# KLab/YAIK

Measured on AMD Instinct MI355X. Metric: Mpix/s tile encode (alpha reject + 7 gradient passes + 8x8 range quant), 8K RGBA, higher is better.
Workload: dtype u8/int32 (+f32 mode-selection sums)

## Files before the change

### yaik_amd/csrc/yk_encode2.hip

```cpp
#include "yk_common.h"
#include "yk_curves.h"
#include "yk_device.h"
#include <mutex>

__constant__ float c_curve2[6][16] = YK_CURVE_TABLE;

#define LS YK_LSTRIDE
#ifdef YK_TEST_HOOKS
#define YK2_ABLATE(bit) ((P.ablate & (bit)) != 0)
#else
#define YK2_ABLATE(bit) false
#endif

__device__ __forceinline__ int y2_byte(uint32_t w, int ch) { return (w >> (8 * ch)) & 255; }
__device__ __forceinline__ uint32_t y2_absdiff(uint32_t a, uint32_t b) { uint32_t r; asm("v_sad_u32 %0, %1, %2, 0" : "=v"(r) : "v"(a), "v"(b)); return r; }
__device__ __forceinline__ int y2_round6(int v) { return (v & ~3) | (v >> 6); }
__device__ __forceinline__ int y2_round6p(int v) { v = min(v + 1, 255); return (v & ~3) | (v >> 6); }

typedef short y2s2 __attribute__((ext_vector_type(2)));
typedef unsigned short y2u2 __attribute__((ext_vector_type(2)));
__device__ __forceinline__ y2u2 y2_u2(uint32_t w) { return __builtin_bit_cast(y2u2, w); }
__device__ __forceinline__ y2s2 y2_s2(y2u2 v) { return __builtin_bit_cast(y2s2, v); }
__device__ __forceinline__ y2u2 y2_splat(int v) { const unsigned short t = (unsigned short)v; return (y2u2){ t, t }; }
__device__ __forceinline__ y2s2 y2_splats(int v) { const short t = (short)v; return (y2s2){ t, t }; }
__device__ __forceinline__ y2s2 y2_rg(uint32_t p) { return y2_s2(y2_u2(__builtin_amdgcn_perm(0u, p, 0x010C000Cu) ^ 0x80008000u)); }
__device__ __forceinline__ y2s2 y2_bb(uint32_t pEven, uint32_t pOdd) { return y2_s2(y2_u2(__builtin_amdgcn_perm(pOdd, pEven, 0x060C020Cu) ^ 0x80008000u)); }
#define YK2_LATN 85
#ifdef YK2_STATS
__device__ unsigned long long g_y2_stats[128];
#define YK2_STAT(i, n) do { if (lane == 0) atomicAdd(&g_y2_stats[(i)], (unsigned long long)(n)); } while (0)
extern "C" int yk_debug_path_stats(unsigned long long* out, int clear) {
    hipError_t e = hipMemcpyFromSymbol(out, HIP_SYMBOL(g_y2_stats), sizeof(g_y2_stats));
    if (e == hipSuccess && clear) { static unsigned long long z[128]; e = hipMemcpyToSymbol(HIP_SYMBOL(g_y2_stats), z, sizeof(z)); }
    return (int)e;
}
#else
#define YK2_STAT(i, n) do { } while (0)
#endif

__device__ __forceinline__ constexpr int y2_cell_x(int m) { return (m & 1) | ((m >> 1) & 2); }
__device__ __forceinline__ constexpr int y2_cell_y(int m) { return ((m >> 1) & 1) | ((m >> 2) & 2); }
template <int NX, int NY> __device__ __forceinline__ constexpr unsigned long long y2_origin() {
    unsigned long long m = 0;
    for (int i = 0; i < 16; i++) if ((y2_cell_x(i) % NX) == 0 && (y2_cell_y(i) % NY) == 0) m |= 1ULL << i;
    return m * 0x0001000100010001ULL;
}
template <int NX, int NY> __device__ __forceinline__ unsigned long long y2_fold(unsigned long long m) {
    if (NX >= 2) m |= m >> 1;
    if (NY >= 2) m |= m >> 2;
    if (NX == 4) m |= m >> 4;
    if (NY == 4) m |= m >> 8;
    return m;
}
template <int NX, int NY> __device__ __forceinline__ unsigned long long y2_spread(unsigned long long m) {
    if (NX >= 2) m |= m << 1;
    if (NY >= 2) m |= m << 2;
    if (NX == 4) m |= m << 4;
    if (NY == 4) m |= m << 8;
    return m;
}

template <int SX, int SY, bool SMOOTH = false>
__device__ __forceinline__ void y2_grad_pass(const uint32_t* s_lat, const int lat, const int cx, const int cy,
                                             const y2s2 (&rg)[16], const y2s2 (&bb)[8], unsigned long long& cov, const unsigned long long deadLanes, const bool stripInside,
                                             const int gxCell, const int gyCell, const int w, const int h, const int rf,
                                             uint32_t* s_bm, const int bxCell, const int byCell, const uint32_t* s_pix, uint8_t* s_list, uint32_t* s_tf, const int lane) {
    constexpr int TX = 1 << SX, TY = 1 << SY, NX = TX / 4, NY = TY / 4;
    constexpr unsigned long long ORG = y2_origin<NX, NY>();
    const int dcx = cx & (NX - 1), dcy = cy & (NY - 1);
    unsigned long long viable = ORG & ~cov & ~y2_fold<NX, NY>(deadLanes);
    if (!stripInside) {
        const int tgx = gxCell - dcx * 4, tgy = gyCell - dcy * 4;
        viable &= __ballot((tgx + TX <= w) && (tgy + TY <= h));
    }
    if (viable == 0ULL) return;
    constexpr int kPassId = (SX == 4 && SY == 4) ? 0 : (SX == 4 && SY == 3) ? 1 : (SX == 3 && SY == 4) ? 2 : (SX == 3 && SY == 3) ? 3 : (SX == 3 && SY == 2) ? 4 : (SX == 2 && SY == 3) ? 5 : 6;
    YK2_STAT(kPassId * 10 + 0, 1); YK2_STAT(kPassId * 10 + 8, __popcll(y2_spread<NX, NY>(viable)));
    const int loO = -256 * rf, hiO = 256 * rf + 255;
    const y2s2 loO2 = y2_splats(loO), hiO2 = y2_splats(hiO), loR2 = y2_splats(loO - 127), hiR2 = y2_splats(hiO - 127);


#ifndef YK2_NO_COMPACT
    const unsigned long long cells = y2_spread<NX, NY>(viable);
    const int nCells = __popcll(cells);
    if (nCells <= 16) {
        YK2_STAT(kPassId * 10 + 1, 1); YK2_STAT(kPassId * 10 + 7, nCells);
        const int rank = (int)__builtin_amdgcn_mbcnt_hi((uint32_t)(cells >> 32), __builtin_amdgcn_mbcnt_lo((uint32_t)cells, 0u));
        const bool mine = __builtin_amdgcn_inverse_ballot_w64(cells);
        if (mine) s_list[rank] = (uint8_t)lane;
        s_tf[lane] = 0u; s_tf[64 + lane] = 0u;
        __builtin_amdgcn_fence(__ATOMIC_RELEASE, "wavefront"); __builtin_amdgcn_wave_barrier(); __builtin_amdgcn_fence(__ATOMIC_ACQUIRE, "wavefront");
        const int j = lane & 15, r = lane >> 4;
        const bool act = j < nCells;
        const int c = (int)s_list[act ? j : 0];
        const int q2 = c >> 4, cy2 = y2_cell_y(c & 15), cx2 = y2_cell_x(c & 15);
        const int dcx2 = cx2 & (NX - 1), dcy2 = cy2 & (NY - 1);
        constexpr int kInTile = (NX > 1 ? 1 : 0) | (NY > 1 ? 2 : 0) | (NX > 2 ? 4 : 0) | (NY > 2 ? 8 : 0);
        const int orig = c & ~kInTile;
        const int lo2 = cy2 * 17 + q2 * 4 + cx2 - dcy2 * 17 - dcx2;
        const y2u2 wyr = y2_splat(16 - ((dcy2 * 4 + r) << (4 - SY)));
        const y2u2 lxc = y2_splat(16 - ((dcx2 * 4) << (4 - SX)));
        const uint4 pr = *reinterpret_cast<const uint4*>(&s_pix[(cy2 * 4 + r) * LS + q2 * 16 + cx2 * 4]);
        const y2s2 rgc[4] = { y2_rg(pr.x), y2_rg(pr.y), y2_rg(pr.z), y2_rg(pr.w) }, bbc[2] = { y2_bb(pr.x, pr.y), y2_bb(pr.z, pr.w) };
        y2s2 mnc[5], mxc[5];
        auto rowC = [&](const unsigned mask) {
            y2u2 Sc[5], stc[5];
#pragma unroll
            for (int t = 0; t < 5; t++) {
                if (!((mask >> t) & 1u)) continue;
                const uint32_t* lt = s_lat + t * YK2_LATN + lo2;
                const y2u2 TL = y2_u2(lt[0]), TR = y2_u2(lt[NX]), BL = y2_u2(lt[NY * 17]), BR = y2_u2(lt[NY * 17 + NX]);
                const y2u2 e16 = (BL - BR) << 4, g = TR - BR, f = TL - BL - g;
                const y2u2 c2 = (g << 4) + f * lxc;
                Sc[t] = ((BR << 8) + e16 * lxc + c2 * wyr) ^ y2_splat(0x8000);
                stc[t] = (e16 + f * wyr) << (4 - SX);
            }
#pragma unroll
            for (int i = 0; i < 4; i++) {
                const y2s2 c01 = rgc[i], cb = bbc[i >> 1];
                const y2s2 cc[4] = { __builtin_shufflevector(c01, c01, 0, 0), __builtin_shufflevector(c01, c01, 1, 1),
                                     (i & 1) ? __builtin_shufflevector(cb, cb, 1, 1) : __builtin_shufflevector(cb, cb, 0, 0), c01 };
#pragma unroll
                for (int t = 0; t < 4; t++) {
                    if (!((mask >> t) & 1u)) continue;
                    const y2s2 D = __builtin_elementwise_sub_sat(y2_s2(Sc[t]), cc[t]);
                    if (i == 0) { mnc[t] = D; mxc[t] = D; }
                    else { mnc[t] = __builtin_elementwise_min(mnc[t], D); mxc[t] = __builtin_elementwise_max(mxc[t], D); }
                    if (i < 3) Sc[t] = Sc[t] - stc[t];
                }
            }
            if (mask & 0x10u) {
                const y2s2 Da = __builtin_elementwise_sub_sat(y2_s2(Sc[4] - stc[4] * (y2u2){ 0, 1 }), bbc[0]);
                const y2s2 Db = __builtin_elementwise_sub_sat(y2_s2(Sc[4] - stc[4] * (y2u2){ 2, 3 }), bbc[1]);
                mnc[4] = __builtin_elementwise_min(Da, Db); mxc[4] = __builtin_elementwise_max(Da, Db);
            }
        };
        constexpr uint32_t kAllFail = 0xE000E000u;
        auto failBits = [&](const y2s2 mnA, const y2s2 mxA, const y2s2 mnP, const y2s2 mxP) -> uint32_t {
            const y2s2 zero = y2_splats(0);
            const y2s2 oA = __builtin_elementwise_sub_sat(zero, __builtin_elementwise_max(__builtin_elementwise_sub_sat(loO2, mnA), __builtin_elementwise_sub_sat(mxA, hiO2)));
            const y2s2 rA = __builtin_elementwise_sub_sat(zero, __builtin_elementwise_max(__builtin_elementwise_sub_sat(loR2, mnA), __builtin_elementwise_sub_sat(mxA, hiR2)));
            const y2s2 oP = __builtin_elementwise_sub_sat(zero, __builtin_elementwise_max(__builtin_elementwise_sub_sat(loO2, mnP), __builtin_elementwise_sub_sat(mxP, hiO2)));
            const y2s2 rP = __builtin_elementwise_sub_sat(zero, __builtin_elementwise_max(__builtin_elementwise_sub_sat(loR2, mnP), __builtin_elementwise_sub_sat(mxP, hiR2)));
            const uint32_t a = __builtin_bit_cast(uint32_t, oA), b = __builtin_bit_cast(uint32_t, rA), cO = __builtin_bit_cast(uint32_t, oP), cR = __builtin_bit_cast(uint32_t, rP);
            uint32_t m = (a & 0x80008000u) | ((b >> 1) & 0x40004000u);
            m |= (((cO << 16) | cO) >> 2) & 0x20000000u;
            m |= (((cR >> 16) | cR) >> 2) & 0x00002000u;
            return m;
        };
        rowC(0x09u);
        if (act) atomicOr(&s_tf[orig], failBits(mnc[0], mxc[0], mnc[3], mxc[3]));
        __builtin_amdgcn_fence(__ATOMIC_RELEASE, "wavefront"); __builtin_amdgcn_wave_barrier(); __builtin_amdgcn_fence(__ATOMIC_ACQUIRE, "wavefront");
        const unsigned long long alive = viable & __ballot(s_tf[lane] != kAllFail);
        if (alive == 0ULL) { YK2_STAT(100 + kPassId, 1); return; }
        rowC(0x16u);
        {
            const y2s2 mnA = __builtin_elementwise_min(__builtin_elementwise_min(mnc[0], mnc[1]), mnc[2]), mxA = __builtin_elementwise_max(__builtin_elementwise_max(mxc[0], mxc[1]), mxc[2]);
            const y2s2 mnP = __builtin_elementwise_min(mnc[3], mnc[4]), mxP = __builtin_elementwise_max(mxc[3], mxc[4]);
            if (act) atomicOr(&s_tf[64 + orig], failBits(mnA, mxA, mnP, mxP));
        }
        __builtin_amdgcn_fence(__ATOMIC_RELEASE, "wavefront"); __builtin_amdgcn_wave_barrier(); __builtin_amdgcn_fence(__ATOMIC_ACQUIRE, "wavefront");
        const unsigned long long acceptC = alive & __ballot(s_tf[64 + lane] != kAllFail);
        if (acceptC != 0ULL) {
            YK2_STAT(110 + kPassId, 1);
            cov |= y2_spread<NX, NY>(acceptC);
            if (__builtin_amdgcn_inverse_ballot_w64(acceptC)) {
                const int tbx = bxCell >> SX, tby = byCell >> SY;
                int bit;
                if (SX == 4 && SY == 4) bit = 0 + tby * 4 + tbx;
                else if (SX == 4 && SY == 3) bit = 32 + tby * 4 + tbx;
                else if (SX == 3 && SY == 4) bit = 64 + tby * 8 + tbx;
                else if (SX == 3 && SY == 3) bit = 96 + tby * 8 + tbx;
                else if (SX == 3 && SY == 2) bit = 160 + (tby >> 3) * 64 + (tby & 7) * 8 + tbx;
                else if (SX == 2 && SY == 3) bit = 288 + (tbx >> 3) * 64 + tby * 8 + (tbx & 7);
                else bit = 416 + ((tby >> 3) * 2 + (tbx >> 3)) * 64 + (tby & 7) * 8 + (tbx & 7);
                atomicOr(&s_bm[bit >> 5], 1u << (bit & 31));
            }
        }
        return;
    }
#endif

    const int lo = lat - dcy * 17 - dcx;
    const y2u2 wy2 = y2_splat(16 - ((dcy * 4) << (4 - SY)));
    const y2u2 lx2 = y2_splat(16 - ((dcx * 4) << (4 - SX)));
    y2u2 S[4], st[4], dS0[4], dS3[4], dst[4], Sa, Sb, rsA, rsB;
    auto setup = [&](const int t) {
        const uint32_t* lt = s_lat + t * YK2_LATN + lo;
        const y2u2 TL = y2_u2(lt[0]), TR = y2_u2(lt[NX]), BL = y2_u2(lt[NY * 17]), BR = y2_u2(lt[NY * 17 + NX]);
        const y2u2 e16 = (BL - BR) << 4, g = TR - BR, f = TL - BL - g;
        const y2u2 c2 = (g << 4) + f * lx2;
        const y2u2 s0 = ((BR << 8) + e16 * lx2 + c2 * wy2) ^ y2_splat(0x8000);
        const y2u2 d0 = c2 << (4 - SY);
        const y2u2 sx = (e16 + f * wy2) << (4 - SX);
        const y2u2 dx = f << (8 - SX - SY);
        if (t < 4) {
            S[t] = s0; dS0[t] = d0; st[t] = sx; dst[t] = dx;
            dS3[t] = d0 - dx * (unsigned short)3;
        } else {
            const y2u2 k01 = { 0, 1 }, k23 = { 2, 3 };
            Sa = s0 - sx * k01; Sb = s0 - sx * k23;
            rsA = d0 - dx * k01; rsB = d0 - dx * k23;
        }
    };
    y2s2 mn[5], mx[5];
    auto pixelRow = [&](const int r, const unsigned mask, const bool first) {
        if (mask & 0x0Fu) {
#pragma unroll
            for (int ii = 0; ii < 4; ii++) {
                const int i = (r & 1) ? 3 - ii : ii;
                const y2s2 c01 = rg[r * 4 + i], cb = bb[r * 2 + (i >> 1)];
                const y2s2 cc[4] = { __builtin_shufflevector(c01, c01, 0, 0), __builtin_shufflevector(c01, c01, 1, 1),
                                     (i & 1) ? __builtin_shufflevector(cb, cb, 1, 1) : __builtin_shufflevector(cb, cb, 0, 0), c01 };
#pragma unroll
                for (int t = 0; t < 4; t++) {
                    if (!((mask >> t) & 1u)) continue;
                    const y2s2 D = __builtin_elementwise_sub_sat(y2_s2(S[t]), cc[t]);
                    if (first && ii == 0) { mn[t] = D; mx[t] = D; }
                    else { mn[t] = __builtin_elementwise_min(mn[t], D); mx[t] = __builtin_elementwise_max(mx[t], D); }
                    if (ii < 3) S[t] = (r & 1) ? S[t] + st[t] : S[t] - st[t];
                }
            }
        }
        if (mask & 0x10u) {
            const y2s2 Da = __builtin_elementwise_sub_sat(y2_s2(Sa), bb[r * 2]), Db = __builtin_elementwise_sub_sat(y2_s2(Sb), bb[r * 2 + 1]);
            const y2s2 lo4 = __builtin_elementwise_min(Da, Db), hi4 = __builtin_elementwise_max(Da, Db);
            if (first) { mn[4] = lo4; mx[4] = hi4; }
            else { mn[4] = __builtin_elementwise_min(mn[4], lo4); mx[4] = __builtin_elementwise_max(mx[4], hi4); }
        }
    };
    auto nextRow = [&](const int r, const unsigned mask) {
#pragma unroll
        for (int t = 0; t < 4; t++) if ((mask >> t) & 1u) { S[t] -= (r & 1) ? dS0[t] : dS3[t]; st[t] -= dst[t]; }
        if (mask & 0x10u) { Sa -= rsA; Sb -= rsB; }
    };
    auto failA4 = [&](const y2s2 mnA, const y2s2 mxA) -> unsigned long long {
        const y2s2 oA = __builtin_elementwise_max(__builtin_elementwise_sub_sat(loO2, mnA), __builtin_elementwise_sub_sat(mxA, hiO2));
        const y2s2 rA = __builtin_elementwise_max(__builtin_elementwise_sub_sat(loR2, mnA), __builtin_elementwise_sub_sat(mxA, hiR2));
        unsigned long long f = y2_fold<NX, NY>(__ballot(oA.x > 0));
        f &= y2_fold<NX, NY>(__ballot(oA.y > 0));
        f &= y2_fold<NX, NY>(__ballot(rA.x > 0));
        f &= y2_fold<NX, NY>(__ballot(rA.y > 0));
        return f;
    };
    auto failP2 = [&](const y2s2 mnP, const y2s2 mxP) -> unsigned long long {
        const y2s2 oP = __builtin_elementwise_max(__builtin_elementwise_sub_sat(loO2, mnP), __builtin_elementwise_sub_sat(mxP, hiO2));
        const y2s2 rP = __builtin_elementwise_max(__builtin_elementwise_sub_sat(loR2, mnP), __builtin_elementwise_sub_sat(mxP, hiR2));
        return y2_fold<NX, NY>(__ballot((oP.x > 0) | (oP.y > 0))) & y2_fold<NX, NY>(__ballot((rP.x > 0) | (rP.y > 0)));
    };
    auto mnAll = [&]() { return __builtin_elementwise_min(__builtin_elementwise_min(mn[0], mn[1]), mn[2]); };
    auto mxAll = [&]() { return __builtin_elementwise_max(__builtin_elementwise_max(mx[0], mx[1]), mx[2]); };

    constexpr bool kScreen = (NX * NY >= 4);
    constexpr unsigned kA = 0x07u, kP = 0x18u;
    unsigned long long accept;
    if (SMOOTH) {
        setup(0); setup(1); setup(2);
        pixelRow(0, kA, true);
        nextRow(0, kA); pixelRow(1, kA, false);
        nextRow(1, kA); pixelRow(2, kA, false);
        nextRow(2, kA); pixelRow(3, kA, false);
// ... 3 lines not shown
        {
            y2u2 S_[4], st_[4], a_[4], b_[4], c_[4]; y2s2 mn_[5], mx_[5];
            for (int t = 0; t < 4; t++) { S_[t] = S[t]; st_[t] = st[t]; a_[t] = dS0[t]; b_[t] = dS3[t]; c_[t] = dst[t]; }
            for (int t = 0; t < 5; t++) { mn_[t] = mn[t]; mx_[t] = mx[t]; }
            setup(3); setup(4);
            pixelRow(0, kP, true); nextRow(0, kP); pixelRow(1, kP, false); nextRow(1, kP); pixelRow(2, kP, false); nextRow(2, kP); pixelRow(3, kP, false);
            const unsigned long long accP = viable & ~failP2(__builtin_elementwise_min(mn[3], mn[4]), __builtin_elementwise_max(mx[3], mx[4]));
            YK2_STAT(97, __popcll(accept)); YK2_STAT(98, __popcll(accP)); YK2_STAT(99, __popcll(accept | accP)); YK2_STAT(96 + 0 * kPassId, 0);
            YK2_STAT(107, __popcll(viable));
            for (int t = 0; t < 4; t++) { S[t] = S_[t]; st[t] = st_[t]; dS0[t] = a_[t]; dS3[t] = b_[t]; dst[t] = c_[t]; }
            for (int t = 0; t < 5; t++) { mn[t] = mn_[t]; mx[t] = mx_[t]; }
        }
#endif
        const unsigned long long rest = viable & ~accept;
        if (rest != 0ULL) {
            YK2_STAT(kPassId * 10 + 5, 1); YK2_STAT(90 + kPassId, __popcll(y2_spread<NX, NY>(rest)));
            setup(3);
            pixelRow(0, 0x08u, true);
            const unsigned long long left = rest & ~failP2(mn[3], mx[3]);
            if (left != 0ULL) {
                setup(4);
                pixelRow(0, 0x10u, true);
                nextRow(0, kP); pixelRow(1, kP, false);
                nextRow(1, kP); pixelRow(2, kP, false);
                nextRow(2, kP); pixelRow(3, kP, false);
                accept |= left & ~failP2(__builtin_elementwise_min(mn[3], mn[4]), __builtin_elementwise_max(mx[3], mx[4]));
            }
        }
    } else {
    int pRows;
    if (kScreen) {
        setup(0); setup(3);
        pixelRow(0, 0x09u, true);
        viable &= ~(failA4(mn[0], mx[0]) & failP2(mn[3], mx[3]));
        if (viable == 0ULL) { YK2_STAT(kPassId * 10 + 2, 1); return; }
        setup(1); setup(2);
        pixelRow(0, 0x06u, true);
        viable &= ~(failA4(mnAll(), mxAll()) & failP2(mn[3], mx[3]));
        if (viable == 0ULL) { YK2_STAT(kPassId * 10 + 3, 1); return; }
        nextRow(0, kA);
        pixelRow(1, kA, false);
        pRows = 0;
    } else {
#pragma unroll
        for (int t = 0; t < 5; t++) setup(t);
        pixelRow(0, 0x1Fu, true);
        viable &= ~(failA4(mnAll(), mxAll()) & failP2(__builtin_elementwise_min(mn[3], mn[4]), __builtin_elementwise_max(mx[3], mx[4])));
        if (viable == 0ULL) { YK2_STAT(kPassId * 10 + 3, 1); return; }
        nextRow(0, 0x1Fu);
        pixelRow(1, 0x1Fu, false);
        if (NX * NY <= 2) {
            viable &= ~(failA4(mnAll(), mxAll()) & failP2(__builtin_elementwise_min(mn[3], mn[4]), __builtin_elementwise_max(mx[3], mx[4])));
            if (viable == 0ULL) { YK2_STAT(kPassId * 10 + 9, 1); return; }
        }
        pRows = 2;
    }
    YK2_STAT(kPassId * 10 + 4, 1);
    nextRow(1, kA);
    pixelRow(2, kA, false);
    nextRow(2, kA);
    pixelRow(3, kA, false);
    accept = viable & ~failA4(mnAll(), mxAll());
    const unsigned long long rest = viable & ~accept;
    if (rest != 0ULL) {
        YK2_STAT(kPassId * 10 + 5, 1); YK2_STAT(90 + kPassId, __popcll(y2_spread<NX, NY>(rest)));
        if (kScreen) {
            setup(4);
            pixelRow(0, 0x10u, true);
            nextRow(0, kP);
            pixelRow(1, kP, false);
        }
        nextRow(1, kP);
        pixelRow(2, kP, false);
        nextRow(2, kP);
        pixelRow(3, kP, false);
        accept |= rest & ~failP2(__builtin_elementwise_min(mn[3], mn[4]), __builtin_elementwise_max(mx[3], mx[4]));
    }
    (void)pRows;
    }
    if (accept == 0ULL) return;
    YK2_STAT(kPassId * 10 + 6, 1);
    cov |= y2_spread<NX, NY>(accept);
    if (__builtin_amdgcn_inverse_ballot_w64(accept)) {
        const int tbx = bxCell >> SX, tby = byCell >> SY;
        int bit;
        if (SX == 4 && SY == 4) bit = 0 + tby * 4 + tbx;
        else if (SX == 4 && SY == 3) bit = 32 + tby * 4 + tbx;
        else if (SX == 3 && SY == 4) bit = 64 + tby * 8 + tbx;
        else if (SX == 3 && SY == 3) bit = 96 + tby * 8 + tbx;
        else if (SX == 3 && SY == 2) bit = 160 + (tby >> 3) * 64 + (tby & 7) * 8 + tbx;
        else if (SX == 2 && SY == 3) bit = 288 + (tbx >> 3) * 64 + tby * 8 + (tbx & 7);
        else bit = 416 + ((tby >> 3) * 2 + (tbx >> 3)) * 64 + (tby & 7) * 8 + (tbx & 7);
        atomicOr(&s_bm[bit >> 5], 1u << (bit & 31));
    }
}

#define YK2_QROWS 258
#define YK2_QR0 32
#define YK2_QNR 224
#define YK2_QBYTES ((size_t)YK2_QNR * YK2_QROWS * 16)
#define YK2_RCPBYTES ((size_t)256 * sizeof(float))
#define YK2_DEFN1 224
#define YK2_DEFBYTES ((size_t)225 * YK2_DEFN1 * 4)
#define YK2_TABBYTES (YK2_QBYTES + YK2_RCPBYTES + YK2_DEFBYTES)
typedef _Float16 y2h2 __attribute__((ext_vector_type(2)));
__device__ __forceinline__ uint32_t y2_f16_bits(int n) { const _Float16 h = (_Float16)(float)n; return (uint32_t)__builtin_bit_cast(unsigned short, h); }
__global__ void yk_qtab_kernel(uint4* tab) {
    __shared__ int K[6][16];
    const int R = YK2_QR0 + (int)blockIdx.x, t = threadIdx.x;
    if (t < 96) { const int m = t >> 4, i = t & 15; K[m][i] = __float2int_rz(__fmul_rn(c_curve2[m][i], (float)R)); }
    __syncthreads();
    if (t < YK2_QROWS) {
        const int o = t - 2;
        uint32_t md[6], idx = 0;
        for (int m = 0; m < 6; m++) {
            const int cnt = m < 3 ? 16 : 8;
            int best = 1 << 30, bi = 0;
            for (int n = 0; n < cnt; n++) { const int d = abs(K[m][n] - o); if (d < best) { best = d; bi = n; } }
            best = min(best, 255);
            md[m] = y2_f16_bits(best);
            idx |= (uint32_t)bi << (4 * m);
        }
        tab[(size_t)blockIdx.x * YK2_QROWS + t] = make_uint4(md[0] | (md[1] << 16), md[2] | (md[3] << 16), md[4] | (md[5] << 16), idx);
    }
}
struct Y2TileDef { int base, BN, dist, R; };
__device__ __forceinline__ Y2TileDef y2_tile_def(const int min_, const int d8) {
    Y2TileDef d;
    d.base = (min_ * 63 + 112) / 224;
    d.BN = (d.base * 224) / 63;
    const int scale = 223 - d.BN;
    const int dnum = (d8 - 32) * 127 + (scale - 1);
    d.dist = (scale < 0) ? -dnum : dnum / scale;
    d.R = (d.dist * scale) / 127 + 32;
    return d;
}
__global__ void yk_deftab_kernel(uint32_t* tab) {
    const int min_ = blockIdx.x, d8 = 32 + (int)threadIdx.x;
    const Y2TileDef d = y2_tile_def(min_, d8);
    const int R = min(max(d.R, YK2_QR0), YK2_QR0 + YK2_QNR - 1);
    const uint32_t rowBase = (uint32_t)((R - YK2_QR0) * YK2_QROWS + 2 - d.BN + 256);
    tab[min_ * YK2_DEFN1 + (int)threadIdx.x] = rowBase | (((((uint32_t)d.dist & 255u) << 7) | ((uint32_t)d.base & 255u)) << 16);
}

__global__ void yk_selftest_qtab_kernel(const uint4* tab, const uint32_t* deftab, int* mismatches) {
    const int mn = blockIdx.x, mx = threadIdx.x;
    if (mx < mn) return;
    const int min_ = min(mn, 224);
    int diff = mx - min_; if (diff < 16) diff = 16;
    const int d8 = max(diff, 32);
    const Y2TileDef d = y2_tile_def(min_, d8);
    const int BN = d.BN, R = d.R;
    int bad = 0;
    if (R < YK2_QR0 || R >= YK2_QR0 + YK2_QNR || mn - BN < -2) { atomicAdd(mismatches, 1); return; }
    {
        const uint32_t e = deftab[min_ * YK2_DEFN1 + (d8 - 32)];
        if ((e & 0xFFFFu) != (uint32_t)((R - YK2_QR0) * YK2_QROWS + 2 - BN + 256)) bad++;
        if ((e >> 16) != ((((uint32_t)d.dist & 255u) << 7) | ((uint32_t)d.base & 255u))) bad++;
    }
    for (int m = 0; m < 6; m++) {
        const int cnt = m < 3 ? 16 : 8;
        int L[16];
        for (int i = 0; i < cnt; i++) {
            L[i] = __float2int_rz(__fadd_rn((float)BN, __fmul_rn(c_curve2[m][i], (float)R)));
            if (L[i] != BN + __float2int_rz(__fmul_rn(c_curve2[m][i], (float)R))) bad++;
        }
        for (int v = mn; v <= mx; v++) {
            int best = 1 << 30, bi = 0;
            for (int n = 0; n < cnt; n++) { const int dd = abs(L[n] - v); if (dd < best) { best = dd; bi = n; } }
            const uint4 row = tab[(size_t)(R - YK2_QR0) * YK2_QROWS + (v - BN + 2)];
            const uint32_t w = m < 2 ? row.x : (m < 4 ? row.y : row.z);
            const uint32_t hb = (m & 1) ? (w >> 16) : (w & 0xFFFFu);
            const int ix = (row.w >> (4 * m)) & 15;
            if (hb != y2_f16_bits(best) || ix != bi) bad++;
        }
    }
    if (bad) atomicAdd(mismatches, bad);
// ... 118 lines not shown
    const int32_t* const boundsP = P.bounds ? P.bounds + fr * 16 : nullptr;
    uint8_t* const slotsP = P.slots + fr * P.fs.slots;
    uint32_t* const blockCntP = P.blockCnt + fr * P.fs.blockN;
    const int BY = L / P.xBB64, BX = L - BY * P.xBB64;
    const int w = P.w, h = P.h;

    YK2_PROBE(0);
    if (lane < 24) s_bm[lane] = 0;
    {
        const int g4 = (lane & 15) * 4, r0 = lane >> 4;
        const int gx = BX * 64 + g4;
        const bool inX = gx + 3 < w;
        const int gxc = min(gx, w - 4);
        const int gyS = BY * 64 + wave * 16;
        const int gyB = min(gyS, P.hAvail - 1);
        const size_t rowBase = (size_t)gyB * (size_t)P.strideElems;
        const char* const b0 = reinterpret_cast<const char*>(pl0 + rowBase);
        const char* const b1 = reinterpret_cast<const char*>(pl1 + rowBase);
        const char* const b2 = reinterpret_cast<const char*>(pl2 + rowBase);
        int4 R[4], G[4], B[4];
#pragma unroll
        for (int k = 0; k < 4; k++) {
            const int rel = min(gyS + r0 + 4 * k, P.hAvail - 1) - gyB;
            const uint32_t off = (uint32_t)(rel * P.strideElems + gxc) * 4u;
            R[k] = *reinterpret_cast<const int4*>(b0 + off);
            G[k] = *reinterpret_cast<const int4*>(b1 + off);
            B[k] = *reinterpret_cast<const int4*>(b2 + off);
        }
        int4 Rb, Gb, Bb;
        {
            const int rel = min(gyS + 16, P.hAvail - 1) - gyB;
            const uint32_t off = (uint32_t)(rel * P.strideElems + gxc) * 4u;
            Rb = *reinterpret_cast<const int4*>(b0 + off);
            Gb = *reinterpret_cast<const int4*>(b1 + off);
            Bb = *reinterpret_cast<const int4*>(b2 + off);
        }
        uint32_t hcol;
        const int hr = min(max(lane - 32, 0), 16);
        {
            const int rel = min(gyS + hr, P.hAvail - 1) - gyB;
            const uint32_t off = (uint32_t)(rel * P.strideElems + min(BX * 64 + 64, w - 1)) * 4u;
            hcol = y2_pack3(*reinterpret_cast<const int32_t*>(b0 + off), *reinterpret_cast<const int32_t*>(b1 + off), *reinterpret_cast<const int32_t*>(b2 + off));
        }
        const float4 rc4 = *reinterpret_cast<const float4*>(P.qtab + YK2_QBYTES + (size_t)lane * 16);

        __builtin_amdgcn_s_setprio(0);
        uint4 o[4], ob;
#pragma unroll
        for (int k = 0; k < 4; k++) {
            o[k] = make_uint4(y2_pack3(R[k].x, G[k].x, B[k].x), y2_pack3(R[k].y, G[k].y, B[k].y), y2_pack3(R[k].z, G[k].z, B[k].z), y2_pack3(R[k].w, G[k].w, B[k].w));
            *reinterpret_cast<uint4*>(&s_pix[(r0 + 4 * k) * LS + g4]) = o[k];
        }
        ob = make_uint4(y2_pack3(Rb.x, Gb.x, Bb.x), y2_pack3(Rb.y, Gb.y, Bb.y), y2_pack3(Rb.z, Gb.z, Bb.z), y2_pack3(Rb.w, Gb.w, Bb.w));
        if (lane < 16) *reinterpret_cast<uint4*>(&s_pix[16 * LS + g4]) = ob;
        if (BX * 64 + 64 > w) {
            if (!inX) {
#pragma unroll
                for (int k = 0; k < 4; k++) *reinterpret_cast<uint4*>(&s_pix[(r0 + 4 * k) * LS + g4]) = make_uint4(o[k].w, o[k].w, o[k].w, o[k].w);
                if (lane < 16) *reinterpret_cast<uint4*>(&s_pix[16 * LS + g4]) = make_uint4(ob.w, ob.w, ob.w, ob.w);
            }
        }
        if (lane >= 32 && lane <= 48) s_pix[hr * LS + 64] = hcol;
        *reinterpret_cast<float4*>(&s_rcp[lane * 4]) = rc4;

    }
    __syncthreads();
    YK2_PROBE(1);

    const int q = lane >> 4, cx = y2_cell_x(lane & 15), cy = y2_cell_y(lane & 15);
    const int bxCell = q * 16 + cx * 4, byCell = wave * 16 + cy * 4;
    const int gxCell = BX * 64 + bxCell, gyCell = BY * 64 + byCell;
    const int lcell = (cy * 4) * LS + bxCell;
    const int lat = cy * 17 + q * 4 + cx;
    const bool mtIn = (BX * 64 + q * 16 < w) && (BY * 64 + wave * 16 < h);

    uint32_t pw[16];
#pragma unroll
    for (int r = 0; r < 4; r++) {
        const uint4 t = *reinterpret_cast<const uint4*>(&s_pix[lcell + r * LS]);
        pw[r * 4 + 0] = t.x; pw[r * 4 + 1] = t.y; pw[r * 4 + 2] = t.z; pw[r * 4 + 3] = t.w;
    }

    unsigned long long cov = 0ULL;
    {
        bool dead = !mtIn;
        {
            const int lim = 4 * P.rejectFactor + 1;
            const y2u2 rb0 = y2_u2(pw[0] & 0x00FF00FFu), rb1 = y2_u2(pw[1] & 0x00FF00FFu), rb2 = y2_u2(pw[2] & 0x00FF00FFu), rb3 = y2_u2(pw[3] & 0x00FF00FFu);
            const y2u2 ga = y2_u2(__builtin_amdgcn_perm(pw[1], pw[0], 0x0C050C01u)), gb = y2_u2(__builtin_amdgcn_perm(pw[2], pw[1], 0x0C050C01u)),
                       gc = y2_u2(__builtin_amdgcn_perm(pw[3], pw[2], 0x0C050C01u));
            const y2u2 l2 = y2_splat(lim);
            const y2u2 u1 = rb0 + rb2 - rb1 - rb1 + l2, u2 = rb1 + rb3 - rb2 - rb2 + l2, ug = ga + gc - gb - gb + l2;
            const y2u2 um = __builtin_elementwise_max(__builtin_elementwise_max(u1, u2), ug);
            dead |= __builtin_bit_cast(uint32_t, __builtin_elementwise_sub_sat(um, y2_splat(2 * lim))) != 0u;
        }
        const unsigned long long deadLanes = __ballot(dead);
        YK2_STAT(75, 1); YK2_STAT(76, ~deadLanes == 0ULL ? 1 : 0); YK2_STAT(77, __popcll(deadLanes));
        const bool stripInside = (BX * 64 + 64 <= w) && (BY * 64 + wave * 16 + 16 <= h);
        if (~deadLanes != 0ULL && !YK2_ABLATE(2)) {
            auto latticePoint = [&](const int idx) {
                const int lr = (idx * 241) >> 12, lc = idx - lr * 17;
                const uint32_t raw = s_pix[(lr * 4) * LS + lc * 4];
                const uint32_t r6 = (raw & 0x00FCFCFCu) | ((raw >> 6) & 0x00030303u);
                const uint32_t z = (raw & 0x007F7F7Fu) + 0x00010101u;
                const uint32_t inc = (z ^ (raw & 0x00808080u)) | (((z & raw & 0x00808080u) >> 7) * 255u);
                const uint32_t p6 = (inc & 0x00FCFCFCu) | ((inc >> 6) & 0x00030303u);
                s_lat[0 * YK2_LATN + idx] = __builtin_amdgcn_perm(r6, raw, 0x0C040C00u);
                s_lat[1 * YK2_LATN + idx] = __builtin_amdgcn_perm(r6, raw, 0x0C050C01u);
                s_lat[2 * YK2_LATN + idx] = __builtin_amdgcn_perm(r6, raw, 0x0C060C02u);
                s_lat[3 * YK2_LATN + idx] = __builtin_amdgcn_perm(p6, p6, 0x0C010C00u);
                s_lat[4 * YK2_LATN + idx] = __builtin_amdgcn_perm(p6, p6, 0x0C020C02u);
            };
            latticePoint(lane);
            if (lane < YK2_LATN - 64) latticePoint(lane + 64);
            __syncthreads();
            y2s2 rg[16], bb[8];
#pragma unroll
            for (int k = 0; k < 16; k++) rg[k] = y2_rg(pw[k]);
#pragma unroll
            for (int k = 0; k < 8; k++) bb[k] = y2_bb(pw[2 * k], pw[2 * k + 1]);
            if (deadLanes == 0ULL) y2_grad_pass<4, 4, true>(s_lat, lat, cx, cy, rg, bb, cov, deadLanes, stripInside, gxCell, gyCell, w, h, P.rejectFactor, s_bm, bxCell, byCell, s_pix, s_list, s_range, lane);
            else y2_grad_pass<4, 4>(s_lat, lat, cx, cy, rg, bb, cov, deadLanes, stripInside, gxCell, gyCell, w, h, P.rejectFactor, s_bm, bxCell, byCell, s_pix, s_list, s_range, lane);
            if (~(cov | deadLanes) != 0ULL) {
                y2_grad_pass<4, 3>(s_lat, lat, cx, cy, rg, bb, cov, deadLanes, stripInside, gxCell, gyCell, w, h, P.rejectFactor, s_bm, bxCell, byCell, s_pix, s_list, s_range, lane);
                y2_grad_pass<3, 4>(s_lat, lat, cx, cy, rg, bb, cov, deadLanes, stripInside, gxCell, gyCell, w, h, P.rejectFactor, s_bm, bxCell, byCell, s_pix, s_list, s_range, lane);
                y2_grad_pass<3, 3>(s_lat, lat, cx, cy, rg, bb, cov, deadLanes, stripInside, gxCell, gyCell, w, h, P.rejectFactor, s_bm, bxCell, byCell, s_pix, s_list, s_range, lane);
                y2_grad_pass<3, 2>(s_lat, lat, cx, cy, rg, bb, cov, deadLanes, stripInside, gxCell, gyCell, w, h, P.rejectFactor, s_bm, bxCell, byCell, s_pix, s_list, s_range, lane);
                y2_grad_pass<2, 3>(s_lat, lat, cx, cy, rg, bb, cov, deadLanes, stripInside, gxCell, gyCell, w, h, P.rejectFactor, s_bm, bxCell, byCell, s_pix, s_list, s_range, lane);
                y2_grad_pass<2, 2>(s_lat, lat, cx, cy, rg, bb, cov, deadLanes, stripInside, gxCell, gyCell, w, h, P.rejectFactor, s_bm, bxCell, byCell, s_pix, s_list, s_range, lane);
            }
#pragma unroll
            for (int r = 0; r < 4; r++) {
                const uint4 t = *reinterpret_cast<const uint4*>(&s_pix[lcell + r * LS]);
                pw[r * 4 + 0] = t.x; pw[r * 4 + 1] = t.y; pw[r * 4 + 2] = t.z; pw[r * 4 + 3] = t.w;
            }
        }
    }
    const int mtIdx = ((BY * 64 + wave * 16) >> 4) * P.mtW + ((BX * 64 + q * 16) >> 4);
    __syncthreads();
    YK2_PROBE(2);
    uint8_t* const small = P.small;
    const uint32_t bmv = s_bm[lane < 24 ? lane : 0];
    auto bmWord = [&](const int k) -> uint32_t { return (uint32_t)__builtin_amdgcn_readlane((int)bmv, k); };
    const uint32_t i64 = (uint32_t)(BY * P.xBB64 + BX);
    const uint32_t frU = (uint32_t)fr;
    uint32_t off32 = ~0u, val32 = 0u;
    {
        const uint32_t w1 = (uint32_t)wave & 1u, w2 = (uint32_t)wave >> 1;
        uint32_t off8 = 0u, val8 = 0u;
        off8 = y2_writelane(P.oBm0b + frU * (uint32_t)P.fs.bm0b + i64 * 4u + (uint32_t)wave, 0, off8);
        val8 = y2_writelane((bmWord(0) >> (4 * wave)) & 0xFu, 0, val8);
        off8 = y2_writelane(P.oBm[1] + frU * (uint32_t)P.fs.bitmap[1] + i64 * 4u + (uint32_t)wave, 1, off8);
        val8 = y2_writelane(bmWord(1) >> (8 * wave), 1, val8);
        off8 = y2_writelane(P.oBm[2] + frU * (uint32_t)P.fs.bitmap[2] + i64 * 4u + (uint32_t)wave, 2, off8);
        val8 = y2_writelane(bmWord(2) >> (8 * wave), 2, val8);
        if (lane < 3) Y2_STORE_IF(8, *(small + off8), (uint8_t)val8);
        const unsigned long long t = ((cov >> 2) ^ cov) & 0x0C0C0C0C0C0C0C0CULL;
        const unsigned long long covRM = cov ^ t ^ (t << 2);
        uint32_t off16 = ((lane & 15) == 0 && mtIn) ? P.oCov + (frU * (uint32_t)P.fs.coverage + (uint32_t)mtIdx) * 2u : ~0u;
        uint32_t val16 = (uint32_t)((covRM >> (q * 16)) & 0xFFFFULL);
        off16 = y2_writelane(P.oBm[3] + frU * (uint32_t)P.fs.bitmap[3] + (i64 * 4u + (uint32_t)wave) * 2u, 1, off16);
        val16 = y2_writelane(bmWord(3 + (int)w2) >> (16 * w1), 1, val16);
#pragma unroll
        for (int sx = 0; sx < 2; sx++) {
            const bool in = BX * 2 + sx < P.xBB32;
            off16 = y2_writelane(in ? P.oBm[5] + frU * (uint32_t)P.fs.bitmap[5] + ((uint32_t)((BY * P.xBB32 + BX * 2 + sx) * 4 + wave)) * 2u : ~0u, 2 + sx, off16);
            val16 = y2_writelane(bmWord(9 + sx * 2 + (int)w2) >> (16 * w1), 2 + sx, val16);
        }
        if (off16 != ~0u) Y2_STORE_IF(8, *reinterpret_cast<uint16_t*>(small + off16), (uint16_t)val16);
        if (P.pixCache != nullptr) {
            const bool cellIn = (gxCell < w) && (gyCell < h);
            if (cellIn && !((cov >> lane) & 1ULL)) {
                const uint32_t strip = (uint32_t)((BY * 4 + wave) * P.xBB64 + BX);
                uint4* dstp = P.pixCache + (size_t)strip * 256 + lane;
#pragma unroll
                for (int r = 0; r < 4; r++) dstp[r * 64] = make_uint4(pw[r * 4 + 0], pw[r * 4 + 1], pw[r * 4 + 2], pw[r * 4 + 3]);
            }
        }
        {
            const bool in = BY * 2 + (int)w2 < P.yBB32;
            off32 = y2_writelane(in ? P.oBm[4] + frU * (uint32_t)P.fs.bitmap[4] + ((uint32_t)(((BY * 2 + (int)w2) * P.xBB64 + BX) * 2) + w1) * 4u : ~0u, 1, off32);
            val32 = y2_writelane(bmWord(5 + (int)w2 * 2 + (int)w1), 1, val32);
#pragma unroll
            for (int sx = 0; sx < 2; sx++) {
                const bool in6 = in && (BX * 2 + sx < P.xBB32);
                off32 = y2_writelane(in6 ? P.oBm[6] + frU * (uint32_t)P.fs.bitmap[6] + ((uint32_t)(((BY * 2 + (int)w2) * P.xBB32 + BX * 2 + sx) * 2) + w1) * 4u : ~0u, 2 + sx, off32);
                val32 = y2_writelane(bmWord(13 + ((int)w2 * 2 + sx) * 2 + (int)w1), 2 + sx, val32);
            }
        }
    }
    YK2_PROBE(3);
    int cxB = 0, cyB = 0, cw = w, chh = P.fullH, discard = 1;
    if (boundsP) {
        const int b0 = boundsP[0], b1 = boundsP[1], b2 = boundsP[2], b3 = boundsP[3];
        discard = (b0 == 0 && b1 == 0 && b2 == w && b3 == P.fullH) ? 1 : 0;
        cxB = (b0 >> 3) << 3; cyB = (b1 >> 3) << 3;
        cw = (((b2 + 7) >> 3) << 3) - cxB; chh = (((b3 + 7) >> 3) << 3) - cyB;
    }
    const int cxl = cx & 1, cyl = cy & 1;
    const int tgx = gxCell - cxl * 4, tgyl = gyCell - cyl * 4, tgy = tgyl + P.y0;
    const bool tileIn = (tgx + 8 <= w) && (tgyl + 8 <= h);
    const bool part = tileIn && tgx >= cxB && tgx < cxB + cw && tgy >= cyB && tgy < cyB + chh && (tgx + 8 <= cw) && (tgy + 8 <= chh);
    const bool keepMT = (keepP == nullptr) || discard || (mtIn && keepP[mtIdx] != 0);
    const bool tileLive = part && keepMT;
    const int l00 = lane & ~3;
    const uint32_t quadN = (uint32_t)((~cov) >> l00) & 15u;
    const int v00 = (int)(quadN & 1u), v01 = (int)((quadN >> 2) & 1u);
    const bool valid = tileLive && ((quadN >> (lane & 3)) & 1u);
    const int nTop = __popc(quadN & 3u), nBot = __popc(quadN >> 2);
    const int tileIdx = (tgyl >> 3) * P.tilesW + (tgx >> 3);
    const size_t T8 = (size_t)P.tilesW * P.tilesH;
    const int tw = lane >> 2;
// ... 424 lines not shown
```

Measured before the change: 231,700.

## Co-schedule next gradient pass cells into the compact 16-lane evaluation

When the compact path of passes 3x3, 3x2 and 2x3 has spare lanes, the candidate cells of the following pass are appended to the same list and evaluated together. Their fail bits are packed into the same words, shifted by three. Cells already evaluated this way are skipped via an `evaluated` mask in the next pass. This aims to cut the number of serial pass invocations and barriers per wave for sparse leftovers. In exchange it adds per-lane dynamic offsets and shifts, so some values that were compile-time constants now vary by lane, and it adds bookkeeping and extra wave barriers.

```diff
diff --git a/yaik_amd/csrc/yk_encode2.hip b/yaik_amd/csrc/yk_encode2.hip
--- a/yaik_amd/csrc/yk_encode2.hip
+++ b/yaik_amd/csrc/yk_encode2.hip
@@ -27,11 +27,11 @@
 __device__ __forceinline__ y2s2 y2_bb(uint32_t pEven, uint32_t pOdd) { return y2_s2(y2_u2(__builtin_amdgcn_perm(pOdd, pEven, 0x060C020Cu) ^ 0x80008000u)); }
 #define YK2_LATN 85
 #ifdef YK2_STATS
-__device__ unsigned long long g_y2_stats[128];
+__device__ unsigned long long g_y2_stats[192];
 #define YK2_STAT(i, n) do { if (lane == 0) atomicAdd(&g_y2_stats[(i)], (unsigned long long)(n)); } while (0)
 extern "C" int yk_debug_path_stats(unsigned long long* out, int clear) {
     hipError_t e = hipMemcpyFromSymbol(out, HIP_SYMBOL(g_y2_stats), sizeof(g_y2_stats));
-    if (e == hipSuccess && clear) { static unsigned long long z[128]; e = hipMemcpyToSymbol(HIP_SYMBOL(g_y2_stats), z, sizeof(z)); }
+    if (e == hipSuccess && clear) { static unsigned long long z[192]; e = hipMemcpyToSymbol(HIP_SYMBOL(g_y2_stats), z, sizeof(z)); }
     return (int)e;
 }
 #else
@@ -60,19 +60,38 @@
     return m;
 }
 
+__device__ __forceinline__ constexpr int y2_pass_sx(int id) { return id < 2 ? 4 : (id < 5 ? 3 : 2); }
+__device__ __forceinline__ constexpr int y2_pass_sy(int id) { return id == 0 || id == 2 ? 4 : (id == 1 || id == 3 || id == 5 ? 3 : 2); }
+template <int SX, int SY> __device__ __forceinline__ unsigned long long y2_viable(const unsigned long long cov, const unsigned long long deadLanes, const bool stripInside,
+                                                                                  const int cx, const int cy, const int gxCell, const int gyCell, const int w, const int h) {
+    constexpr int TX = 1 << SX, TY = 1 << SY, NX = TX / 4, NY = TY / 4;
+    unsigned long long viable = y2_origin<NX, NY>() & ~cov & ~y2_fold<NX, NY>(deadLanes);
+    if (!stripInside) {
+        const int tgx = gxCell - (cx & (NX - 1)) * 4, tgy = gyCell - (cy & (NY - 1)) * 4;
+        viable &= __ballot((tgx + TX <= w) && (tgy + TY <= h));
+    }
+    return viable;
+}
+template <int SX, int SY> __device__ __forceinline__ int y2_bitmap_bit(const int bxCell, const int byCell) {
+    const int tbx = bxCell >> SX, tby = byCell >> SY;
+    if (SX == 4 && SY == 4) return 0 + tby * 4 + tbx;
+    if (SX == 4 && SY == 3) return 32 + tby * 4 + tbx;
+    if (SX == 3 && SY == 4) return 64 + tby * 8 + tbx;
+    if (SX == 3 && SY == 3) return 96 + tby * 8 + tbx;
+    if (SX == 3 && SY == 2) return 160 + (tby >> 3) * 64 + (tby & 7) * 8 + tbx;
+    if (SX == 2 && SY == 3) return 288 + (tbx >> 3) * 64 + tby * 8 + (tbx & 7);
+    return 416 + ((tby >> 3) * 2 + (tbx >> 3)) * 64 + (tby & 7) * 8 + (tbx & 7);
+}
+
 template <int SX, int SY, bool SMOOTH = false>
 __device__ __forceinline__ void y2_grad_pass(const uint32_t* s_lat, const int lat, const int cx, const int cy,
-                                             const y2s2 (&rg)[16], const y2s2 (&bb)[8], unsigned long long& cov, const unsigned long long deadLanes, const bool stripInside,
+                                             const y2s2 (&rg)[16], const y2s2 (&bb)[8], unsigned long long& cov, unsigned long long& evaluated, const unsigned long long deadLanes, const bool stripInside,
                                              const int gxCell, const int gyCell, const int w, const int h, const int rf,
                                              uint32_t* s_bm, const int bxCell, const int byCell, const uint32_t* s_pix, uint8_t* s_list, uint32_t* s_tf, const int lane) {
     constexpr int TX = 1 << SX, TY = 1 << SY, NX = TX / 4, NY = TY / 4;
-    constexpr unsigned long long ORG = y2_origin<NX, NY>();
     const int dcx = cx & (NX - 1), dcy = cy & (NY - 1);
-    unsigned long long viable = ORG & ~cov & ~y2_fold<NX, NY>(deadLanes);
-    if (!stripInside) {
-        const int tgx = gxCell - dcx * 4, tgy = gyCell - dcy * 4;
-        viable &= __ballot((tgx + TX <= w) && (tgy + TY <= h));
-    }
+    unsigned long long viable = y2_viable<SX, SY>(cov, deadLanes, stripInside, cx, cy, gxCell, gyCell, w, h) & ~evaluated;
+    evaluated = 0ULL;
     if (viable == 0ULL) return;
     constexpr int kPassId = (SX == 4 && SY == 4) ? 0 : (SX == 4 && SY == 3) ? 1 : (SX == 3 && SY == 4) ? 2 : (SX == 3 && SY == 3) ? 3 : (SX == 3 && SY == 2) ? 4 : (SX == 2 && SY == 3) ? 5 : 6;
     YK2_STAT(kPassId * 10 + 0, 1); YK2_STAT(kPassId * 10 + 8, __popcll(y2_spread<NX, NY>(viable)));
@@ -85,21 +104,64 @@
     const int nCells = __popcll(cells);
     if (nCells <= 16) {
         YK2_STAT(kPassId * 10 + 1, 1); YK2_STAT(kPassId * 10 + 7, nCells);
+        constexpr bool kHasNext = kPassId >= 3 && kPassId <= 5;
+        constexpr int SXB = kHasNext ? y2_pass_sx(kPassId + 1) : SX, SYB = kHasNext ? y2_pass_sy(kPassId + 1) : SY;
+        constexpr int NXB = (1 << SXB) / 4, NYB = (1 << SYB) / 4;
+        unsigned long long viableB = 0ULL, cellsB = 0ULL;
+        int nB = 0;
+#if !defined(YK2_NO_GROUP) || defined(YK2_STATS)
+        if (kHasNext) {
+            viableB = y2_viable<SXB, SYB>(cov, deadLanes, stripInside, cx, cy, gxCell, gyCell, w, h);
+            cellsB = y2_spread<NXB, NYB>(viableB);
+            nB = __popcll(cellsB);
+#ifdef YK2_STATS
+            {
+                constexpr int k = kPassId - 3;
+                constexpr int SXC = y2_pass_sx(kPassId <= 4 ? kPassId + 2 : 6), SYC = y2_pass_sy(kPassId <= 4 ? kPassId + 2 : 6);
+                int n2 = 0, n3 = 0;
+                if (kPassId <= 4) n2 = __popcll(y2_spread<(1 << SXC) / 4, (1 << SYC) / 4>(y2_viable<SXC, SYC>(cov, deadLanes, stripInside, cx, cy, gxCell, gyCell, w, h)));
+                if (kPassId == 3) n3 = __popcll(y2_viable<2, 2>(cov, deadLanes, stripInside, cx, cy, gxCell, gyCell, w, h));
+                if (nB > 0) {
+                    YK2_STAT(136 + k, 1);
+                    if (nCells + nB <= 16) YK2_STAT(130 + k, 1);
+                    if (kPassId <= 4 && n2 > 0 && nCells + nB + n2 <= 16) YK2_STAT(133 + k, 1);
+                    if (kPassId == 3 && n2 > 0 && n3 > 0 && nCells + nB + n2 + n3 <= 16) YK2_STAT(135, 1);
+                }
+            }
+#endif
+#ifdef YK2_NO_GROUP
+            nB = 0;
+#endif
+            if (nB == 0 || nCells + nB > 16) { viableB = 0ULL; cellsB = 0ULL; nB = 0; }
+        }
+#endif
         const int rank = (int)__builtin_amdgcn_mbcnt_hi((uint32_t)(cells >> 32), __builtin_amdgcn_mbcnt_lo((uint32_t)cells, 0u));
         const bool mine = __builtin_amdgcn_inverse_ballot_w64(cells);
         if (mine) s_list[rank] = (uint8_t)lane;
+        if (kHasNext && nB != 0) {
+            YK2_STAT(140 + kPassId - 3, 1); YK2_STAT(150 + kPassId - 3, nB);
+            const int rankB = (int)__builtin_amdgcn_mbcnt_hi((uint32_t)(cellsB >> 32), __builtin_amdgcn_mbcnt_lo((uint32_t)cellsB, 0u));
+            if (__builtin_amdgcn_inverse_ballot_w64(cellsB)) s_list[nCells + rankB] = (uint8_t)lane;
+        }
         s_tf[lane] = 0u; s_tf[64 + lane] = 0u;
         __builtin_amdgcn_fence(__ATOMIC_RELEASE, "wavefront"); __builtin_amdgcn_wave_barrier(); __builtin_amdgcn_fence(__ATOMIC_ACQUIRE, "wavefront");
         const int j = lane & 15, r = lane >> 4;
-        const bool act = j < nCells;
+        const bool act = j < nCells + nB;
+        const bool isB = kHasNext && j >= nCells;
         const int c = (int)s_list[act ? j : 0];
         const int q2 = c >> 4, cy2 = y2_cell_y(c & 15), cx2 = y2_cell_x(c & 15);
-        const int dcx2 = cx2 & (NX - 1), dcy2 = cy2 & (NY - 1);
         constexpr int kInTile = (NX > 1 ? 1 : 0) | (NY > 1 ? 2 : 0) | (NX > 2 ? 4 : 0) | (NY > 2 ? 8 : 0);
-        const int orig = c & ~kInTile;
+        constexpr int kInTileB = (NXB > 1 ? 1 : 0) | (NYB > 1 ? 2 : 0) | (NXB > 2 ? 4 : 0) | (NYB > 2 ? 8 : 0);
+        const int nxL = isB ? NXB : NX, nyL = isB ? NYB : NY;
+        const int shx = isB ? 4 - SXB : 4 - SX, shy = isB ? 4 - SYB : 4 - SY;
+        const int dcx2 = cx2 & (nxL - 1), dcy2 = cy2 & (nyL - 1);
+        const int orig = c & ~(isB ? kInTileB : kInTile);
+        const int fsh = isB ? 3 : 0;
         const int lo2 = cy2 * 17 + q2 * 4 + cx2 - dcy2 * 17 - dcx2;
-        const y2u2 wyr = y2_splat(16 - ((dcy2 * 4 + r) << (4 - SY)));
-        const y2u2 lxc = y2_splat(16 - ((dcx2 * 4) << (4 - SX)));
+        const int oTR = nxL, oBL = nyL * 17;
+        const y2u2 wyr = y2_splat(16 - ((dcy2 * 4 + r) << shy));
+        const y2u2 lxc = y2_splat(16 - ((dcx2 * 4) << shx));
+        const y2u2 shx2 = y2_splat(shx);
         const uint4 pr = *reinterpret_cast<const uint4*>(&s_pix[(cy2 * 4 + r) * LS + q2 * 16 + cx2 * 4]);
         const y2s2 rgc[4] = { y2_rg(pr.x), y2_rg(pr.y), y2_rg(pr.z), y2_rg(pr.w) }, bbc[2] = { y2_bb(pr.x, pr.y), y2_bb(pr.z, pr.w) };
         y2s2 mnc[5], mxc[5];
@@ -109,11 +171,11 @@
             for (int t = 0; t < 5; t++) {
                 if (!((mask >> t) & 1u)) continue;
                 const uint32_t* lt = s_lat + t * YK2_LATN + lo2;
-                const y2u2 TL = y2_u2(lt[0]), TR = y2_u2(lt[NX]), BL = y2_u2(lt[NY * 17]), BR = y2_u2(lt[NY * 17 + NX]);
+                const y2u2 TL = y2_u2(lt[0]), TR = y2_u2(lt[oTR]), BL = y2_u2(lt[oBL]), BR = y2_u2(lt[oBL + oTR]);
                 const y2u2 e16 = (BL - BR) << 4, g = TR - BR, f = TL - BL - g;
                 const y2u2 c2 = (g << 4) + f * lxc;
                 Sc[t] = ((BR << 8) + e16 * lxc + c2 * wyr) ^ y2_splat(0x8000);
-                stc[t] = (e16 + f * wyr) << (4 - SX);
+                stc[t] = (e16 + f * wyr) << shx2;
             }
 #pragma unroll
             for (int i = 0; i < 4; i++) {
@@ -148,35 +210,41 @@
             m |= (((cR >> 16) | cR) >> 2) & 0x00002000u;
             return m;
         };
+        constexpr uint32_t kAllFailB = kAllFail >> 3;
         rowC(0x09u);
-        if (act) atomicOr(&s_tf[orig], failBits(mnc[0], mxc[0], mnc[3], mxc[3]));
+        if (act) atomicOr(&s_tf[orig], failBits(mnc[0], mxc[0], mnc[3], mxc[3]) >> fsh);
         __builtin_amdgcn_fence(__ATOMIC_RELEASE, "wavefront"); __builtin_amdgcn_wave_barrier(); __builtin_amdgcn_fence(__ATOMIC_ACQUIRE, "wavefront");
-        const unsigned long long alive = viable & __ballot(s_tf[lane] != kAllFail);
-        if (alive == 0ULL) { YK2_STAT(100 + kPassId, 1); return; }
+        const uint32_t w1 = s_tf[lane];
+        const unsigned long long alive = viable & __ballot((kHasNext ? (w1 & kAllFail) : w1) != kAllFail);
+        unsigned long long aliveB = 0ULL;
+        if (kHasNext && nB != 0) aliveB = viableB & __ballot((w1 & kAllFailB) != kAllFailB);
+        if ((alive | aliveB) == 0ULL) { YK2_STAT(100 + kPassId, 1); if (nB != 0) { YK2_STAT(146 + kPassId - 3, 1); YK2_STAT(143 + kPassId - 3, 1); } evaluated = viableB; return; }
         rowC(0x16u);
         {
             const y2s2 mnA = __builtin_elementwise_min(__builtin_elementwise_min(mnc[0], mnc[1]), mnc[2]), mxA = __builtin_elementwise_max(__builtin_elementwise_max(mxc[0], mxc[1]), mxc[2]);
             const y2s2 mnP = __builtin_elementwise_min(mnc[3], mnc[4]), mxP = __builtin_elementwise_max(mxc[3], mxc[4]);
-            if (act) atomicOr(&s_tf[64 + orig], failBits(mnA, mxA, mnP, mxP));
+            if (act) atomicOr(&s_tf[64 + orig], failBits(mnA, mxA, mnP, mxP) >> fsh);
         }
         __builtin_amdgcn_fence(__ATOMIC_RELEASE, "wavefront"); __builtin_amdgcn_wave_barrier(); __builtin_amdgcn_fence(__ATOMIC_ACQUIRE, "wavefront");
-        const unsigned long long acceptC = alive & __ballot(s_tf[64 + lane] != kAllFail);
-        if (acceptC != 0ULL) {
-            YK2_STAT(110 + kPassId, 1);
-            cov |= y2_spread<NX, NY>(acceptC);
-            if (__builtin_amdgcn_inverse_ballot_w64(acceptC)) {
-                const int tbx = bxCell >> SX, tby = byCell >> SY;
-                int bit;
-                if (SX == 4 && SY == 4) bit = 0 + tby * 4 + tbx;
-                else if (SX == 4 && SY == 3) bit = 32 + tby * 4 + tbx;
-                else if (SX == 3 && SY == 4) bit = 64 + tby * 8 + tbx;
-                else if (SX == 3 && SY == 3) bit = 96 + tby * 8 + tbx;
-                else if (SX == 3 && SY == 2) bit = 160 + (tby >> 3) * 64 + (tby & 7) * 8 + tbx;
-                else if (SX == 2 && SY == 3) bit = 288 + (tbx >> 3) * 64 + tby * 8 + (tbx & 7);
-                else bit = 416 + ((tby >> 3) * 2 + (tbx >> 3)) * 64 + (tby & 7) * 8 + (tbx & 7);
-                atomicOr(&s_bm[bit >> 5], 1u << (bit & 31));
-            }
-        }
+        const uint32_t w2 = s_tf[64 + lane];
+        const unsigned long long acceptC = alive & __ballot((kHasNext ? (w2 & kAllFail) : w2) != kAllFail);
+        if (acceptC != 0ULL) { YK2_STAT(110 + kPassId, 1); }
+        cov |= y2_spread<NX, NY>(acceptC);
+        unsigned long long acceptB = 0ULL;
+        if (kHasNext && nB != 0) {
+            const unsigned long long stillB = aliveB & ~cov;
+            if (viableB & ~cov) YK2_STAT(143 + kPassId - 3, 1);
+            acceptB = stillB & __ballot((w2 & kAllFailB) != kAllFailB);
+            if (acceptB != 0ULL) { YK2_STAT(153 + kPassId - 3, 1); }
+            cov |= y2_spread<NXB, NYB>(acceptB);
+        }
+        if ((acceptC | acceptB) != 0ULL && __builtin_amdgcn_inverse_ballot_w64(acceptC | acceptB)) {
+            int bit = y2_bitmap_bit<SX, SY>(bxCell, byCell);
+            if (kHasNext && __builtin_amdgcn_inverse_ballot_w64(acceptB)) bit = y2_bitmap_bit<SXB, SYB>(bxCell, byCell);
+            atomicOr(&s_bm[bit >> 5], 1u << (bit & 31));
+        }
+        __builtin_amdgcn_wave_barrier();
+        evaluated = viableB;
         return;
     }
 #endif
@@ -346,17 +414,10 @@
     YK2_STAT(kPassId * 10 + 6, 1);
     cov |= y2_spread<NX, NY>(accept);
     if (__builtin_amdgcn_inverse_ballot_w64(accept)) {
-        const int tbx = bxCell >> SX, tby = byCell >> SY;
-        int bit;
-        if (SX == 4 && SY == 4) bit = 0 + tby * 4 + tbx;
-        else if (SX == 4 && SY == 3) bit = 32 + tby * 4 + tbx;
-        else if (SX == 3 && SY == 4) bit = 64 + tby * 8 + tbx;
-        else if (SX == 3 && SY == 3) bit = 96 + tby * 8 + tbx;
-        else if (SX == 3 && SY == 2) bit = 160 + (tby >> 3) * 64 + (tby & 7) * 8 + tbx;
-        else if (SX == 2 && SY == 3) bit = 288 + (tbx >> 3) * 64 + tby * 8 + (tbx & 7);
-        else bit = 416 + ((tby >> 3) * 2 + (tbx >> 3)) * 64 + (tby & 7) * 8 + (tbx & 7);
+        const int bit = y2_bitmap_bit<SX, SY>(bxCell, byCell);
         atomicOr(&s_bm[bit >> 5], 1u << (bit & 31));
     }
+    __builtin_amdgcn_wave_barrier();
 }
 
 #define YK2_QROWS 258
@@ -641,6 +702,7 @@
     }
 
     unsigned long long cov = 0ULL;
+    unsigned long long evaluated = 0ULL;
     {
         bool dead = !mtIn;
         {
@@ -678,15 +740,15 @@
             for (int k = 0; k < 16; k++) rg[k] = y2_rg(pw[k]);
 #pragma unroll
             for (int k = 0; k < 8; k++) bb[k] = y2_bb(pw[2 * k], pw[2 * k + 1]);
-            if (deadLanes == 0ULL) y2_grad_pass<4, 4, true>(s_lat, lat, cx, cy, rg, bb, cov, deadLanes, stripInside, gxCell, gyCell, w, h, P.rejectFactor, s_bm, bxCell, byCell, s_pix, s_list, s_range, lane);
-            else y2_grad_pass<4, 4>(s_lat, lat, cx, cy, rg, bb, cov, deadLanes, stripInside, gxCell, gyCell, w, h, P.rejectFactor, s_bm, bxCell, byCell, s_pix, s_list, s_range, lane);
+            if (deadLanes == 0ULL) y2_grad_pass<4, 4, true>(s_lat, lat, cx, cy, rg, bb, cov, evaluated, deadLanes, stripInside, gxCell, gyCell, w, h, P.rejectFactor, s_bm, bxCell, byCell, s_pix, s_list, s_range, lane);
+            else y2_grad_pass<4, 4>(s_lat, lat, cx, cy, rg, bb, cov, evaluated, deadLanes, stripInside, gxCell, gyCell, w, h, P.rejectFactor, s_bm, bxCell, byCell, s_pix, s_list, s_range, lane);
             if (~(cov | deadLanes) != 0ULL) {
-                y2_grad_pass<4, 3>(s_lat, lat, cx, cy, rg, bb, cov, deadLanes, stripInside, gxCell, gyCell, w, h, P.rejectFactor, s_bm, bxCell, byCell, s_pix, s_list, s_range, lane);
-                y2_grad_pass<3, 4>(s_lat, lat, cx, cy, rg, bb, cov, deadLanes, stripInside, gxCell, gyCell, w, h, P.rejectFactor, s_bm, bxCell, byCell, s_pix, s_list, s_range, lane);
-                y2_grad_pass<3, 3>(s_lat, lat, cx, cy, rg, bb, cov, deadLanes, stripInside, gxCell, gyCell, w, h, P.rejectFactor, s_bm, bxCell, byCell, s_pix, s_list, s_range, lane);
-                y2_grad_pass<3, 2>(s_lat, lat, cx, cy, rg, bb, cov, deadLanes, stripInside, gxCell, gyCell, w, h, P.rejectFactor, s_bm, bxCell, byCell, s_pix, s_list, s_range, lane);
-                y2_grad_pass<2, 3>(s_lat, lat, cx, cy, rg, bb, cov, deadLanes, stripInside, gxCell, gyCell, w, h, P.rejectFactor, s_bm, bxCell, byCell, s_pix, s_list, s_range, lane);
-                y2_grad_pass<2, 2>(s_lat, lat, cx, cy, rg, bb, cov, deadLanes, stripInside, gxCell, gyCell, w, h, P.rejectFactor, s_bm, bxCell, byCell, s_pix, s_list, s_range, lane);
+                y2_grad_pass<4, 3>(s_lat, lat, cx, cy, rg, bb, cov, evaluated, deadLanes, stripInside, gxCell, gyCell, w, h, P.rejectFactor, s_bm, bxCell, byCell, s_pix, s_list, s_range, lane);
+                y2_grad_pass<3, 4>(s_lat, lat, cx, cy, rg, bb, cov, evaluated, deadLanes, stripInside, gxCell, gyCell, w, h, P.rejectFactor, s_bm, bxCell, byCell, s_pix, s_list, s_range, lane);
+                y2_grad_pass<3, 3>(s_lat, lat, cx, cy, rg, bb, cov, evaluated, deadLanes, stripInside, gxCell, gyCell, w, h, P.rejectFactor, s_bm, bxCell, byCell, s_pix, s_list, s_range, lane);
+                y2_grad_pass<3, 2>(s_lat, lat, cx, cy, rg, bb, cov, evaluated, deadLanes, stripInside, gxCell, gyCell, w, h, P.rejectFactor, s_bm, bxCell, byCell, s_pix, s_list, s_range, lane);
+                y2_grad_pass<2, 3>(s_lat, lat, cx, cy, rg, bb, cov, evaluated, deadLanes, stripInside, gxCell, gyCell, w, h, P.rejectFactor, s_bm, bxCell, byCell, s_pix, s_list, s_range, lane);
+                y2_grad_pass<2, 2>(s_lat, lat, cx, cy, rg, bb, cov, evaluated, deadLanes, stripInside, gxCell, gyCell, w, h, P.rejectFactor, s_bm, bxCell, byCell, s_pix, s_list, s_range, lane);
             }
 #pragma unroll
             for (int r = 0; r < 4; r++) {
```

Result: faster. 234,900, median of 6 (+1.4%).
